# aghasemzadeh/OpenMPL

Hardware: AMD Instinct MI355X
Metric: poses/sec (V=4, J=17, batch=1024 per GPU) fp32 (higher is better)
Workload: dtype f32; 1 GPU; Human3.6M config: V=4 J=17 batch=1024 fp32, CHOSEN flag set, depth 12, DIM 32, heads 8; global_batch=1024, parallelism=single GPU

## Files before the change

openmpl_amd/csrc/spt_native.hip:

```cpp
#include <type_traits>

#include "spt_stage.hpp"

namespace mpl {

constexpr int QS = 100;
constexpr int SPT_LDS_BYTES = (ROWS * XS + ROWS * QS) * 4;

__device__ __forceinline__ int spt_abl(const SptParams& p) {
#ifdef MPL_LAB
    return p.abl;
#else
    return 0;
#endif
}

__device__ __forceinline__ void ln_frags(const float* X, int m, int li, int kq, const float4& g0, const float4& g1,
                                         const float4& b0, const float4& b1, float4& a0, float4& a1) {
    const float* xr = X + (m * 16 + li) * XS + 4 * kq;
    float4 x0 = ld4(xr), x1 = ld4(xr + 16);
    float s = ((x0.x + x0.y) + (x0.z + x0.w)) + ((x1.x + x1.y) + (x1.z + x1.w));
    s = xor16_add(s);
    s = xor32_add(s);
    const float mean = s * (1.0f / 32.0f);
// ... 157 lines not shown
    __device__ __forceinline__ void begin(const mpl_block_weights&, const mpl_block_weights&, bool) {}
};

template <int P, class Weights, class AFrags, class Epilogue>
__device__ __forceinline__ void linear_phase(const Weights& W, int mt, int wave, bool skip, AFrags a_frags, Epilogue epilogue) {
    constexpr int NT = Phase<P>::NT, KH = Phase<P>::KH;
    const int lo = (mt * NT * wave) / NWAVE, hi = (mt * NT * (wave + 1)) / NWAVE;
    for (int m = lo / NT; m * NT < hi && !skip; ++m) {
        float4 a[KH];
        a_frags(m, a);
#pragma unroll
        for (int n = 0; n < NT; ++n) {
            const int u = m * NT + n;
            if (u < lo || u >= hi) continue;
            float4 w[KH];
            float bias;
            W.template tile<P>(n, w, bias);
            f32x4 c = tile_k32(a[0], a[1], w[0], w[1]);
            if constexpr (KH == 4) c = c + tile_k32(a[2], a[3], w[2], w[3]);
            epilogue(m, n, c, bias);
        }
    }
}

template <bool STAGED>
__global__ __launch_bounds__(NTHR, 1) void spt_kernel(const SptParams p) {
    extern __shared__ __attribute__((aligned(1024))) float smem[];
    constexpr int RX = STAGED ? SPT_SMALL_ROWS : ROWS;
    float* WB = smem;
    float* X = smem + (STAGED ? 2 * SPT_WB_FLOATS : 0);
    float* Q = X + RX * XS;

    const int tid = threadIdx.x, lane = tid & 63, wave = __builtin_amdgcn_readfirstlane(tid >> 6);
    const int li = lane & 15, kq = lane >> 4;
    const int view = blockIdx.x % p.V;
    const int b0 = (blockIdx.x / p.V) * p.spw;
    const mpl_spt_set set = p.sets[(p.flags & MPL_F_MULTI_SPT) ? view : 0];
    const float *pose = p.poses[view], *ray = p.rays[view], *cen = p.centers[view];
    const int nl = p.B - b0 < p.spw ? p.B - b0 : p.spw;
    const int rows_live = nl * SJ;
    const int mt = (rows_live + 15) >> 4;

    std::conditional_t<STAGED, StagedWeights, FragWeights> W;
    W.li = li, W.kq = kq;
    if constexpr (STAGED) W.lane = lane;
    mpl_block_weights bw, bw_next;
    if (p.n_apps > 0) {
        bw = set.blocks[p.sched[0] & 0x7f];
        if constexpr (STAGED) stage_block(bw, WB, wave, lane, 0, NWAVE);
        else W.template load<P_QKV>(bw);
        if (STAGED && p.n_apps > 1) bw_next = set.blocks[p.sched[1] & 0x7f];
    }

    spt_embed<false>(p, set, X, tid, b0, pose, ray, cen, nl, mt * 16);
    unsigned char* sched_l = reinterpret_cast<unsigned char*>(WB + SPT_WB_FLOATS + SPT_WB_VEC + 352);
    float* conf_l = WB + SPT_WB_VEC + 352;
    if (STAGED) {
        if (tid < MPL_MAX_APPS) sched_l[tid] = p.sched[tid];
        for (int r = tid; r < rows_live; r += NTHR) {
            const int sq = r / SJ;
            conf_l[r] = pose[((size_t)(b0 + sq) * SJ + (r - sq * SJ)) * 3 + 2];
        }
        asm volatile("s_waitcnt vmcnt(0)" ::: "memory");
    }
    __syncthreads();

    const int abl = spt_abl(p);
    const bool no_mfma = (abl & 4) != 0;
    unsigned long long ph[6] = {0, 0, 0, 0, 0, 0}, tlast = (abl & 16) ? __builtin_amdgcn_s_memtime() : 0;
    auto stamp = [&](int k) {
        if (abl & 16) { const unsigned long long now = __builtin_amdgcn_s_memtime(); ph[k] += now - tlast; tlast = now; }
    };
    float4 g[2], e[2];
    auto a_ln = [&](int m, float4 (&a)[2]) { ln_frags(X, m, li, kq, g[0], g[1], e[0], e[1], a[0], a[1]); };
    auto a_q = [&](int m, auto& a) {
        const float* ar = Q + (m * 16 + li) * QS + 4 * kq;
#pragma unroll
        for (int q = 0; q < (int)(sizeof(a) / sizeof(a[0])); ++q) a[q] = ld4(ar + 16 * q);
    };
    auto add_to_x = [&](int m, int n, const f32x4& c, float b) {
        float* xd = X + (m * 16 + 4 * kq) * XS + n * 16 + li;
#pragma unroll
        for (int r = 0; r < 4; ++r) xd[r * XS] += c[r] + b;
    };
    for (int app = 0; app < p.n_apps; ++app) {
        const bool weighted = ((STAGED ? sched_l[app] : p.sched[app]) & 0x80) != 0;
        const bool more = app + 1 < p.n_apps;
        if (!STAGED && more) bw_next = set.blocks[p.sched[app + 1] & 0x7f];
        if constexpr (STAGED) W.wb = WB + (app & 1) * SPT_WB_FLOATS;
        mpl_block_weights bw_after;

        W.template begin<P_QKV>(bw, bw_next, more);
        W.template ln<P_QKV>(g, e);
        linear_phase<P_QKV>(W, mt, wave, no_mfma, a_ln, [&](int m, int n, const f32x4& c, float b) {
            float* qd = Q + (m * 16 + 4 * kq) * QS + n * 16 + li;
#pragma unroll
            for (int r = 0; r < 4; ++r) qd[r * QS] = c[r] + b;
        });
        __syncthreads();
        stamp(0);

        if (STAGED && more) {
            const int busy = (rows_live * SH + 63) >> 6;
            const int w0 = busy < NWAVE - 1 ? busy : 0;
            stage_block(bw_next, WB + ((app + 1) & 1) * SPT_WB_FLOATS, wave, lane, w0, NWAVE - w0);
            if (app + 2 < p.n_apps) bw_after = set.blocks[sched_l[app + 2] & 0x7f];
        }
        stamp(5);
        for (int pr = tid; pr < rows_live * SH && !(abl & 1); pr += NTHR) {
            const int r = pr >> 3, h = pr & 7;
            const int sq = r / SJ;
            const float* kb = Q + (sq * SJ) * QS + SD + 4 * h;
            const float4 q = ld4(Q + r * QS + 4 * h);
            float sc[SJ];
            float mx = -INFINITY;
#pragma unroll
            for (int j = 0; j < SJ; ++j) {
                const float4 k = ld4(kb + j * QS);
                sc[j] = 0.5f * (fmaf(q.x, k.x, q.y * k.y) + fmaf(q.z, k.z, q.w * k.w));
                mx = fmaxf(mx, sc[j]);
            }
            float l = 0.f;
#pragma unroll
            for (int j = 0; j < SJ; ++j) {
                sc[j] = __expf(sc[j] - mx);
                l += sc[j];
            }
            float inv = 1.0f / l;
            if (weighted) {
                const int b = b0 + sq;
                if (STAGED) inv *= conf_l[r];
                else inv *= (b < p.B) ? pose[((size_t)b * SJ + (r - sq * SJ)) * 3 + 2] : 0.f;
            }
            float4 o = {0.f, 0.f, 0.f, 0.f};
#pragma unroll
            for (int j = 0; j < SJ; ++j) {
                const float4 v = ld4(kb + j * QS + SD);
                const float pj = sc[j] * inv;
                o.x = fmaf(pj, v.x, o.x);
                o.y = fmaf(pj, v.y, o.y);
                o.z = fmaf(pj, v.z, o.z);
                o.w = fmaf(pj, v.w, o.w);
            }
            st4(Q + r * QS + 4 * h, o);
        }
        __syncthreads();
        stamp(1);

        W.template begin<P_PROJ>(bw, bw_next, more);
        linear_phase<P_PROJ>(W, mt, wave, no_mfma, a_q, add_to_x);
        __syncthreads();
        stamp(2);

        W.template begin<P_FC1>(bw, bw_next, more);
        W.template ln<P_FC1>(g, e);
        linear_phase<P_FC1>(W, mt, wave, no_mfma, a_ln, [&](int m, int n, const f32x4& c, float b) {
            float* qd = Q + (m * 16 + 4 * kq) * QS + n * 16 + li;
#pragma unroll
            for (int r = 0; r < 4; ++r) qd[r * QS] = (abl & 2) ? (c[r] + b) : gelu_erf(c[r] + b);
        });
        __syncthreads();
        stamp(3);

        W.template begin<P_FC2>(bw, bw_next, more);
        linear_phase<P_FC2>(W, mt, wave, no_mfma, a_q, add_to_x);
        if (STAGED) asm volatile("s_waitcnt vmcnt(0)" ::: "memory");
        __syncthreads();
        stamp(4);
        bw = bw_next;
        if (STAGED && app + 2 < p.n_apps) bw_next = bw_after;
    }

    if (abl & 16) {
        if (lane == 0 && blockIdx.x < 32) {
            float* o = p.xs + (size_t)(blockIdx.x * NWAVE + wave) * 8;
            for (int k = 0; k < 6; ++k) o[k] = (float)ph[k];
        }
        return;
    }
    spt_epilogue<false>(p, X, tid, view, b0, pose, ray, cen, nl, rows_live);
}

int launch_spt_native(const SptParams& p, int form, int grid, hipStream_t s) {
    if (form == MPL_SPT_STAGED) {
        if (int rc = kernel_lds_once<spt_kernel<true>>(SPT_SMALL_LDS_BYTES)) return rc;
        hipLaunchKernelGGL(spt_kernel<true>, dim3(grid), dim3(NTHR), SPT_SMALL_LDS_BYTES, s, p);
    } else {
        if (int rc = kernel_lds_once<spt_kernel<false>>(SPT_LDS_BYTES)) return rc;
        hipLaunchKernelGGL(spt_kernel<false>, dim3(grid), dim3(NTHR), SPT_LDS_BYTES, s, p);
    }
    return hip_check_launch();
}

}
```

openmpl_amd/csrc/spt_packed.hip:

```cpp
#include "spt_pack.hpp"
#include "spt_stage.hpp"

namespace mpl {

constexpr int ATS = 36;
constexpr int HS = 68;
constexpr int KV_F = SJ * SH * SEQ * 4;
constexpr int SPT3_RING_BYTES = (ROWS * XS + 2 * KV_F + ROWS * ATS) * 4;
constexpr int SPT3_LDS_BYTES = 160 * 1024;
constexpr int SPT3_HID_OFF = 3072;
constexpr int SPT3_Q_OFF = 20480;
static_assert(SPT3_HID_OFF + ROWS * HS <= 2 * KV_F + ROWS * ATS, "HID does not fit its alias");
static_assert((SPT3_HID_OFF + ROWS * HS - 2 * KV_F) * 4 <= SPT3_Q_OFF, "HID reaches into the staged qkv weights");
static_assert(SPT3_Q_OFF + 12 * 1024 <= ROWS * ATS * 4, "staged qkv weights do not fit behind HID in ATT");
static_assert(SPT3_RING_BYTES + 8 * 1024 + 2 * SPT3_NPAR * 4 <= SPT3_LDS_BYTES, "spare LDS too small");

typedef float f32x2 __attribute__((ext_vector_type(2)));

__device__ inline float spt_window_scale(float v) {
    if (!(v > 0.f) || !(v < 3.0e38f)) return 1.0f;
    int e;
    (void)frexpf(32768.0f / v, &e);
    e = e - 1 < -100 ? -100 : (e - 1 > 100 ? 100 : e - 1);
    return ldexpf(1.0f, e);
}

__global__ __launch_bounds__(256) void spt_pack_kernel(const float* __restrict__ qkv_w, const float* __restrict__ qkv_b,
                                                        const float* __restrict__ ln1_w, const float* __restrict__ ln1_b,
                                                        const float* __restrict__ proj_w, const float* __restrict__ proj_b,
                                                        const float* __restrict__ fc1_w, const float* __restrict__ fc1_b,
                                                        const float* __restrict__ ln2_w, const float* __restrict__ ln2_b,
                                                        const float* __restrict__ fc2_w, const float* __restrict__ fc2_b,
                                                        char* __restrict__ dst, int fold_q) {
    __shared__ float Wf[8192];
    __shared__ float cn[SPT_NCOL], sw[SPT_NCOL], bnd[SPT_NCOL], scal[2];
    const int tid = threadIdx.x;
    for (int i = tid; i < 8192; i += 256) {
        float w;
        if (i < 3072) w = qkv_w[i] * ln1_w[i & 31];
        else if (i < 4096) w = proj_w[i - 3072];
        else if (i < 6144) w = fc1_w[i - 4096] * ln2_w[i & 31];
        else w = fc2_w[i - 6144];
        Wf[i] = w;
    }
    __syncthreads();
    if (tid < SPT_NCOL) {
        const int n = tid;
        const float *wr, *raw, *beta = nullptr;
        int K = 32;
        float bias;
        if (n < 96) { wr = Wf + n * 32; raw = qkv_w + n * 32; beta = ln1_b; bias = qkv_b[n]; }
        else if (n < 128) { wr = Wf + 3072 + (n - 96) * 32; raw = proj_w + (n - 96) * 32; bias = proj_b[n - 96]; }
        else if (n < 192) { wr = Wf + 4096 + (n - 128) * 32; raw = fc1_w + (n - 128) * 32; beta = ln2_b; bias = fc1_b[n - 128]; }
        else { wr = Wf + 6144 + (n - 192) * 64; raw = fc2_w + (n - 192) * 64; bias = fc2_b[n - 192]; K = 64; }
        float amax = 0.f;
        double ss = 0.0, c = (double)bias;
        for (int k = 0; k < K; ++k) {
            amax = fmaxf(amax, fabsf(wr[k]));
            ss += (double)wr[k] * (double)wr[k];
            if (beta) c += (double)raw[k] * (double)beta[k];
        }
        float s = 1.0f;
        if (amax > 0.f && amax < 3.0e38f) {
            int e;
            (void)frexpf(amax, &e);
            e = 14 - e;
            e = e < -100 ? -100 : (e > 100 ? 100 : e);
            s = ldexpf(1.0f, e);
// ... 111 lines not shown
            for (int n = 0; n < NCT; ++n) x[n] = res[n];
            if (i + 1 < NM) read_tile(i + 1);
            f32x4 c[NCT];
#pragma unroll
            for (int n = 0; n < NCT; ++n) c[n] = f32x4{0.f, 0.f, 0.f, 0.f};
#pragma unroll
            for (int n = 0; n < NCT; ++n) {
                if (NCT * m + n < LO || NCT * m + n >= HI) continue;
#pragma unroll
                for (int ks = 0; ks < KS; ++ks) c[n] = mfma3(w[n][ks], ah[ks], al[ks], c[n]);
            }
#pragma unroll
            for (int n = 0; n < NCT; ++n) {
                if (NCT * m + n < LO || NCT * m + n >= HI) continue;
                float* dd = d0 + m * 16 * DST + 16 * n;
                if (GELU)
                    st4(dd, float4{gelu_as_scaled(fmaf(c[n][0], sc[n].x, bc[n].x), hs), gelu_as_scaled(fmaf(c[n][1], sc[n].y, bc[n].y), hs),
                                   gelu_as_scaled(fmaf(c[n][2], sc[n].z, bc[n].z), hs), gelu_as_scaled(fmaf(c[n][3], sc[n].w, bc[n].w), hs)});
                else
                    st4(dd, float4{x[n].x + fmaf(c[n][0], sc[n].x, bc[n].x), x[n].y + fmaf(c[n][1], sc[n].y, bc[n].y),
                                   x[n].z + fmaf(c[n][2], sc[n].z, bc[n].z), x[n].w + fmaf(c[n][3], sc[n].w, bc[n].w)});
            }
        }
    }
}
#define SPT_ROLE(W, MTS, KS, LN, GELU, NCT, AST, DST, ...) \
    spt_linear_role<KS, LN, GELU, NCT, AST, DST, ((MTS) * (NCT) * (W)) / NWAVE, ((MTS) * (NCT) * ((W) + 1)) / NWAVE>(__VA_ARGS__)
#define SPT_BY_WAVE(wv, ...)                          \
    switch (wv) {                                     \
        case 0: SPT_ROLE(0, __VA_ARGS__); break;      \
        case 1: SPT_ROLE(1, __VA_ARGS__); break;      \
        case 2: SPT_ROLE(2, __VA_ARGS__); break;      \
        case 3: SPT_ROLE(3, __VA_ARGS__); break;      \
        case 4: SPT_ROLE(4, __VA_ARGS__); break;      \
        case 5: SPT_ROLE(5, __VA_ARGS__); break;      \
        case 6: SPT_ROLE(6, __VA_ARGS__); break;      \
        default: SPT_ROLE(7, __VA_ARGS__); break;     \
    }


template <int SS>
__global__ __launch_bounds__(NTHR, 1) void spt3_kernel(const SptParams p) {
    constexpr int RLIVE = SJ * SS;
    constexpr int MTS = (RLIVE + 15) / 16;
    constexpr int NT = (MTS + 3) / 4;
    extern __shared__ __attribute__((aligned(16))) float smem[];
    float* X = smem;
    float* Kb = smem + ROWS * XS;
    float* Vb = Kb + KV_F;
    float* ATT = Vb + KV_F;
    float* HID = Kb + SPT3_HID_OFF;
    char* S_W = reinterpret_cast<char*>(ATT + ROWS * ATS);
    float* S_PAR = reinterpret_cast<float*>(S_W + 8 * 1024);
    char* R_F1 = reinterpret_cast<char*>(Kb);
    char* R_Q = reinterpret_cast<char*>(ATT) + SPT3_Q_OFF;

    const int tid = threadIdx.x, lane = tid & 63;
    const int wave = __builtin_amdgcn_readfirstlane(tid >> 6);
    const int li = lane & 15, kq = lane >> 4;
    auto phase_sync = [&]() {
        asm volatile("s_waitcnt vmcnt(0)" ::: "memory");
        __syncthreads();
    };
    const int hg = wave & 1, part = wave >> 1;
    const int view = blockIdx.x % p.V;
    const int b0 = (blockIdx.x / p.V) * SS;
    const int sl = li % SS;
    const mpl_spt_set set = p.sets[(p.flags & MPL_F_MULTI_SPT) ? view : 0];
    const float* pose = p.poses[view];
    const float* ray = p.rays[view];
    const float* cen = p.centers[view];

    auto stage_w = [&](char* dst, const unsigned short* pack, int byte_off, int n_pieces) {
        const unsigned l0 = (unsigned)(uintptr_t)(__attribute__((address_space(3))) char*)dst;
        for (int i = wave; i < n_pieces; i += NWAVE)
            ::mpl::dma16(reinterpret_cast<const float*>(reinterpret_cast<const char*>(pack) + byte_off + i * 1024) + lane * 4,
                         l0 + (unsigned)(i * 1024));
    };
    auto load_par = [&](const mpl_block_weights& b) -> float4 {
        if (tid >= SPT3_NPAR / 4) return float4{0.f, 0.f, 0.f, 0.f};
        return ld4(G(reinterpret_cast<const float*>(reinterpret_cast<const char*>(b.qkv_w3) + SPT_PACK_VEC)) + 4 * tid);
    };
    auto store_par = [&](int app_of, const float4& v) {
        if (tid < SPT3_NPAR / 4) st4(S_PAR + (app_of & 1) * SPT3_NPAR + 4 * tid, v);
    };
    mpl_block_weights bw;
    if (p.n_apps > 0) {
        bw = set.blocks[p.sched[0] & 0x7f];
        stage_w(R_Q, bw.qkv_w3, SPT_PACK_QKV, 12);
    }
    const float4 par0 = p.n_apps > 0 ? load_par(bw) : float4{0.f, 0.f, 0.f, 0.f};
    spt_embed<true, SS>(p, set, X, tid, b0, pose, ray, cen, SS, MTS * 16);
    store_par(0, par0);
    phase_sync();

    auto load_w = [&](const char* region, int unit, sf16x8 (&w)[2]) { spt_load_unit(region, unit, lane, w); };
    auto ln_frag = [&](int m, sf16x8& ah, sf16x8& al) {
        const float* xr = X + (m * 16 + li) * XS + 8 * kq;
        spt_ln_split(::mpl::ld4(xr), ::mpl::ld4(xr + 4), ah, al);
    };
    for (int app = 0; app < p.n_apps; ++app) {
        const bool weighted = (p.sched[app] & 0x80) != 0;
        bw = set.blocks[p.sched[app] & 0x7f];
        const unsigned short* pack = bw.qkv_w3;
        const float* par = S_PAR + (app & 1) * SPT3_NPAR;
        stage_w(S_W, pack, SPT_PACK_PROJ, 4);
        {
            sf16x8 wq[3][2];
            float4 bq[3], sq[3];
#pragma unroll
            for (int c = 0; c < 3; ++c) {
                load_w(R_Q, 2 * c + hg, wq[c]);
                bq[c] = ::mpl::ld4(par + SPT_C_QKV + 32 * c + 16 * hg + 4 * kq);
                sq[c] = ::mpl::ld4(par + SPT_NCOL + SPT_C_QKV + 32 * c + 16 * hg + 4 * kq);
            }
            float4 q[NT];
#pragma unroll
            for (int t = 0; t < NT; ++t) {
                q[t] = float4{0.f, 0.f, 0.f, 0.f};
                if (part + 4 * t < MTS && !(p.abl & 8)) {
                    const int m = part + 4 * t;
                    const int j = (16 * m + li) / SS;
                    const bool live = 16 * m + li < RLIVE;
                    sf16x8 ah, al;
                    ln_frag(m, ah, al);
                    const f32x4 z = {0.f, 0.f, 0.f, 0.f};
                    const f32x4 cq = mfma3(wq[0], ah, al, z), ck = mfma3(wq[1], ah, al, z), cv = mfma3(wq[2], ah, al, z);
                    q[t] = float4{fmaf(cq[0], sq[0].x, bq[0].x), fmaf(cq[1], sq[0].y, bq[0].y), fmaf(cq[2], sq[0].z, bq[0].z),
                                  fmaf(cq[3], sq[0].w, bq[0].w)};
                    const int h = 4 * hg + kq;
                    const float kx = fmaf(ck[0], sq[1].x, bq[1].x), ky = fmaf(ck[1], sq[1].y, bq[1].y);
                    const float kz = fmaf(ck[2], sq[1].z, bq[1].z), kw = fmaf(ck[3], sq[1].w, bq[1].w);
                    if (live && j < SJ - 1) {
                        float* kp = Kb + ((((j >> 1) * 2) * SH + h) * SS + sl) * 4 + (j & 1);
                        kp[0] = kx;
                        kp[2] = ky;
                        kp[SH * SS * 4] = kz;
                        kp[SH * SS * 4 + 2] = kw;
                    } else if (live) {
                        st4(Kb + (SJ - 1) * SH * SS * 4 + (h * SS + sl) * 4, float4{kx, ky, kz, kw});
                    }
                    if (live)
                        st4(Vb + ((j * SH + h) * SS + sl) * 4, float4{fmaf(cv[0], sq[2].x, bq[2].x), fmaf(cv[1], sq[2].y, bq[2].y),
                                                                       fmaf(cv[2], sq[2].z, bq[2].z), fmaf(cv[3], sq[2].w, bq[2].w)});
                }
            }
            phase_sync();
            auto attention = [&](auto live_tiles) {
                constexpr int NL = decltype(live_tiles)::value;
                const int h = 4 * hg + kq;
                float sc[NL][SJ];
#pragma unroll
                for (int jp = 0; jp < SJ / 2; ++jp) {
                    const float4 k01 = ::mpl::ld4(Kb + (((jp * 2) * SH + h) * SS + sl) * 4);
                    const float4 k23 = ::mpl::ld4(Kb + (((jp * 2 + 1) * SH + h) * SS + sl) * 4);
                    const f32x2 kx = {k01.x, k01.y}, ky = {k01.z, k01.w}, kz = {k23.x, k23.y}, kw = {k23.z, k23.w};
#pragma unroll
// ... 30 lines not shown
#pragma unroll
                    for (int j = 0; j < SJ; ++j) {
                        sc[t][j] = __builtin_amdgcn_exp2f(sc[t][j] - mx);
                        l += sc[t][j];
                    }
                    inv[t] = __builtin_amdgcn_rcpf(l) * s_att;
                    if (weighted) {
                        const int b = b0 + sl, r = 16 * (part + 4 * t) + li;
                        inv[t] *= (b < p.B && r < RLIVE) ? conf0[3 * (64 / SS) * t] : 0.f;
                    }
                }
                float4 o[NL];
#pragma unroll
                for (int t = 0; t < NL; ++t) o[t] = float4{0.f, 0.f, 0.f, 0.f};
#pragma unroll
                for (int j = 0; j < SJ; ++j) {
                    const float4 v = ::mpl::ld4(Vb + ((j * SH + h) * SS + sl) * 4);
#pragma unroll
                    for (int t = 0; t < NL; ++t) {
                        const float pj = sc[t][j];
                        o[t].x = fmaf(pj, v.x, o[t].x);
                        o[t].y = fmaf(pj, v.y, o[t].y);
                        o[t].z = fmaf(pj, v.z, o[t].z);
                        o[t].w = fmaf(pj, v.w, o[t].w);
                    }
                }
#pragma unroll
                for (int t = 0; t < NL; ++t) {
                    o[t] = float4{o[t].x * inv[t], o[t].y * inv[t], o[t].z * inv[t], o[t].w * inv[t]};
                    if (weighted) {
                        const float big = fmaxf(fmaxf(fabsf(o[t].x), fabsf(o[t].y)), fmaxf(fabsf(o[t].z), fabsf(o[t].w)));
                        if (!(big <= 65000.f)) {
                            const float qn = __builtin_nanf("");
                            o[t] = float4{qn, qn, qn, qn};
                            if (p.err_host) __hip_atomic_fetch_or(p.err_host, 2u, __ATOMIC_RELAXED, __HIP_MEMORY_SCOPE_SYSTEM);
                        }
                    }
                }
#pragma unroll
                for (int t = 0; t < NL; ++t) st4(ATT + ((part + 4 * t) * 16 + li) * ATS + 4 * h, o[t]);
            };
            if (!(p.abl & 1)) {
                if (part + 4 * (NT - 1) < MTS) attention(SptInt<NT>{});
                else if (NT > 1) attention(SptInt<(NT > 1 ? NT - 1 : 1)>{});
            }
        }
        phase_sync();
        stage_w(R_F1, pack, SPT_PACK_FC1, 8);
        if (!(p.abl & 32)) SPT_BY_WAVE(wave, MTS, 1, false, false, 2, ATS, XS, ATT, X, S_W, par, SPT_C_PROJ, 0.f, lane);
        phase_sync();
        stage_w(S_W, pack, SPT_PACK_FC2, 8);
        if (!(p.abl & 64))
            SPT_BY_WAVE(wave, MTS, 1, true, true, 4, XS, HS, X, HID, R_F1, par, SPT_C_FC1, par[2 * SPT_NCOL + 1], lane);
        phase_sync();
        {
            float4 parn = float4{0.f, 0.f, 0.f, 0.f};
            if (app + 1 < p.n_apps) {
                const mpl_block_weights bn = set.blocks[p.sched[app + 1] & 0x7f];
                stage_w(R_Q, bn.qkv_w3, SPT_PACK_QKV, 12);
                parn = load_par(bn);
            }
            if (!(p.abl & 128)) SPT_BY_WAVE(wave, MTS, 2, false, false, 2, HS, XS, HID, X, S_W, par, SPT_C_FC2, 0.f, lane);
            if (app + 1 < p.n_apps) store_par(app + 1, parn);
        }
        phase_sync();
    }
    spt_epilogue<true, SS>(p, X, tid, view, b0, pose, ray, cen, SS, MTS * 16);
}

template <int SS>
static int launch_spt3(const SptParams& p, int grid, hipStream_t s) {
    if (int rc = kernel_lds_once<spt3_kernel<SS>>(SPT3_LDS_BYTES)) return rc;
    hipLaunchKernelGGL(spt3_kernel<SS>, dim3(grid), dim3(NTHR), SPT3_LDS_BYTES, s, p);
    return hip_check_launch();
}

int launch_spt_packed(const SptParams& p, int ss, int grid, hipStream_t s) {
    switch (ss) {
        case 1: return launch_spt3<1>(p, grid, s);
        case 2: return launch_spt3<2>(p, grid, s);
        case 4: return launch_spt3<4>(p, grid, s);
        case 8: return launch_spt3<8>(p, grid, s);
        case 16: return launch_spt3<16>(p, grid, s);
        default: return MPL_E_INVALID;
    }
}

}
```

openmpl_amd/csrc/spt_stage.hpp:

```cpp
#pragma once
#include "common.hpp"

namespace mpl {

constexpr int SJ = 17;
constexpr int SD = 32;
constexpr int SH = 8;
constexpr int SEQ = 16;
constexpr int ROWS = SEQ * SJ;
constexpr int XS = 36;
constexpr int NTHR = 512;
constexpr int NWAVE = NTHR / 64;
constexpr int SPT_SMALL_SPW = 8;

struct SptParams {
    const float* poses[MPL_MAX_VIEWS];
    const float* rays[MPL_MAX_VIEWS];
    const float* centers[MPL_MAX_VIEWS];
    const mpl_spt_set* sets;
    const float *snorm_w, *snorm_b;
    const float *pos3d_embed, *pos3d_view, *pos3d_lin_w, *pos3d_lin_b;
    const float *ray_w, *ray_b, *cfpt_w, *cfpt_b;
    float* xs;
    int B, V, in_ch, n_apps;
    unsigned flags;
    int c3;
    int spw;
    int abl;
    unsigned* err_host;
    unsigned char sched[MPL_MAX_APPS];
};

int launch_spt_native(const SptParams& p, int form, int grid, hipStream_t s);
int launch_spt_packed(const SptParams& p, int ss, int grid, hipStream_t s);

typedef const __attribute__((address_space(1))) float* gfp;
__device__ __forceinline__ gfp G(const float* p) { return (gfp)p; }
__device__ __forceinline__ float4 ld4(gfp p) {
    typedef float v4 __attribute__((ext_vector_type(4)));
    const v4 t = *reinterpret_cast<const __attribute__((address_space(1))) v4*>(p);
    return make_float4(t.x, t.y, t.z, t.w);
}

template <bool TM, int SS = SEQ>
__device__ __forceinline__ void row_to_sj(int r, int& sq, int& j) {
    if (TM) { j = r / SS; sq = r % SS; }
    else { sq = r / SJ; j = r - sq * SJ; }
}

template <bool TM, int SS = SEQ>
__device__ __forceinline__ void spt_embed(const SptParams& p, const mpl_spt_set& set, float* X, int tid, int b0,
                                          const float* pose, const float* ray, const float* cen, int nseq = SEQ, int nrows = ROWS) {
    for (int idx = tid; idx < nrows * SD; idx += NTHR) {
        const int r = idx >> 5, c = idx & 31;
        int sq, j;
        row_to_sj<TM, SS>(r, sq, j);
        const int b = b0 + sq;
        float x = 0.f;
        if (b < p.B && sq < nseq && j < SJ) {
            const float* in = pose + ((size_t)b * SJ + j) * 3;
            const float* we = set.embed_w + c * p.in_ch;
            x = set.embed_b[c] + we[0] * in[0] + we[1] * in[1];
            if (p.in_ch == 3) x += we[2] * in[2];
            if (p.flags & MPL_F_CONF_ADD) x += set.conf_w[c] * in[2] + set.conf_b[c];
            if (p.flags & MPL_F_CONF_MULT) x *= set.conf_w[c] * in[2] + set.conf_b[c];
            x += set.pos_embed[j * SD + c];
            if (p.flags & MPL_F_POS3D_SPATIAL) {
                if (p.flags & MPL_F_POS3D_LEARN) {
                    x += p.pos3d_embed[j * p.c3 + c];
                } else {
                    const float* rr = ray + ((size_t)b * SJ + j) * 3;
                    const float* cc = cen + (size_t)b * 3;
                    const float vx = rr[0] - cc[0], vy = rr[1] - cc[1], vz = rr[2] - cc[2];
                    const float nrm = fmaxf(sqrtf(vx * vx + vy * vy + vz * vz), 1e-12f);
                    const float* wl = p.pos3d_lin_w + c * 3;
                    x += p.pos3d_lin_b[c] + wl[0] * (vx / nrm) + wl[1] * (vy / nrm) + wl[2] * (vz / nrm);
                }
            }
        }
        X[r * XS + c] = x;
    }
}

template <bool TM, int SS = SEQ>
__device__ __forceinline__ void spt_epilogue(const SptParams& p, const float* X, int tid, int view, int b0, const float* pose,
                                             const float* ray, const float* cen, int nseq = SEQ, int nrows = ROWS) {
    const bool to_rays = (p.flags & MPL_F_POS3D_TO_RAYS) && (p.flags & MPL_F_RAYS_TOKEN);
    const bool ray_tok = !(p.flags & MPL_F_POS3D_TO_RAYS) && (p.flags & MPL_F_RAYS_TOKEN);
    const int cw = to_rays ? 2 * SD : SD;
    const int Df = SJ * SD * ((p.flags & MPL_F_RAYS_TOKEN) ? 2 : 1);
    for (int r = tid; r < nrows; r += NTHR) {
        int sq, j;
        row_to_sj<TM, SS>(r, sq, j);
        const int b = b0 + sq;
        if (b >= p.B || sq >= nseq || j >= SJ) continue;
        const float* xr = X + r * XS;
        float v[SD];
        float s = 0.f;
#pragma unroll
        for (int c = 0; c < SD; c += 4) {
            const float4 t = ld4(xr + c);
            v[c] = t.x; v[c + 1] = t.y; v[c + 2] = t.z; v[c + 3] = t.w;
            s += (t.x + t.y) + (t.z + t.w);
        }
        const float mean = s * (1.0f / 32.0f);
        float ss = 0.f;
#pragma unroll
        for (int c = 0; c < SD; ++c) {
            v[c] -= mean;
            ss = fmaf(v[c], v[c], ss);
        }
        const float rstd = 1.0f / sqrtf(ss * (1.0f / 32.0f) + 1e-6f);
        const float conf = pose[((size_t)b * SJ + j) * 3 + 2];
        float dx = 0.f, dy = 0.f, dz = 0.f, nx = 0.f, ny = 0.f, nz = 0.f;
        const bool need_dir = (p.flags & MPL_F_RAYS_TOKEN) ||
                              (!(p.flags & MPL_F_POS3D_SPATIAL) && !(p.flags & MPL_F_POS3D_LEARN));
        if (need_dir) {
            const float* rr = ray + ((size_t)b * SJ + j) * 3;
            const float* cc = cen + (size_t)b * 3;
            dx = rr[0] - cc[0]; dy = rr[1] - cc[1]; dz = rr[2] - cc[2];
            const float nrm = fmaxf(sqrtf(dx * dx + dy * dy + dz * dz), 1e-12f);
            nx = dx / nrm; ny = dy / nrm; nz = dz / nrm;
        }
        auto pos3d = [=](int c) -> float {
            if (p.flags & MPL_F_POS3D_SPATIAL) return p.pos3d_view[j * p.c3 + c];
            if (p.flags & MPL_F_POS3D_LEARN) return p.pos3d_embed[j * p.c3 + c];
            const float* wl = p.pos3d_lin_w + c * 3;
            return p.pos3d_lin_b[c] + wl[0] * nx + wl[1] * ny + wl[2] * nz;
        };
        auto ray_emb = [=](int c) -> float {
            const float* wr = p.ray_w + c * 3;
            return p.ray_b[c] + wr[0] * dx + wr[1] * dy + wr[2] * dz;
        };
        float* orow = p.xs + ((size_t)b * p.V + view) * Df;
        float* o1 = orow + j * cw;
#pragma unroll
        for (int c = 0; c < SD; c += 4) {
            float t[4];
#pragma unroll
            for (int q = 0; q < 4; ++q) {
                float y = v[c + q] * rstd * p.snorm_w[c + q] + p.snorm_b[c + q];
                if (p.flags & MPL_F_CONF_IN_FPT) y += p.cfpt_w[c + q] * conf + p.cfpt_b[c + q];
                t[q] = y + pos3d(c + q);
            }
            st4(o1 + c, float4{t[0], t[1], t[2], t[3]});
        }
        if (to_rays) {
#pragma unroll
            for (int c = 0; c < SD; c += 4) {
                float t[4];
#pragma unroll
                for (int q = 0; q < 4; ++q) t[q] = ray_emb(c + q) + pos3d(SD + c + q);
                st4(o1 + SD + c, float4{t[0], t[1], t[2], t[3]});
            }
        } else if (ray_tok) {
            float* o2 = orow + (SJ + j) * SD;
#pragma unroll
            for (int c = 0; c < SD; c += 4) st4(o2 + c, float4{ray_emb(c), ray_emb(c + 1), ray_emb(c + 2), ray_emb(c + 3)});
        }
    }
}

}
```

Measured before the change: 879,200 poses/s.

## Restructure SPT embed/epilogue for wider parallelism and precompute schedule pointers in LDS

Rewrites the embed stage so each lane holds per-channel weights in registers and processes several rows with batched, prefetched global loads, specialised at compile time by positional-encoding mode. Splits the epilogue into two passes: per-row LayerNorm statistics go to LDS scratch, then 8 threads per row each write a 4-wide slice, so one row is no longer handled serially by a single thread. In the packed kernel, the per-application weight-pack pointers and schedule bytes are resolved once into LDS and read back as scalars, which removes the repeated global lookups of the block table inside the loop. The cost is extra LDS scratch, an added barrier in the epilogue, and higher register pressure.

```diff
diff --git a/openmpl_amd/csrc/spt_native.hip b/openmpl_amd/csrc/spt_native.hip
--- a/openmpl_amd/csrc/spt_native.hip
+++ b/openmpl_amd/csrc/spt_native.hip
@@ -233,6 +233,9 @@
         if (STAGED && p.n_apps > 1) bw_next = set.blocks[p.sched[1] & 0x7f];
     }
 
+    static_assert(MPL_MAX_APPS <= 64, "one lane per scheduled application");
+    unsigned sched_v = 0;
+    if (!STAGED && lane < p.n_apps) sched_v = p.sched[lane];
     spt_embed<false>(p, set, X, tid, b0, pose, ray, cen, nl, mt * 16);
     unsigned char* sched_l = reinterpret_cast<unsigned char*>(WB + SPT_WB_FLOATS + SPT_WB_VEC + 352);
     float* conf_l = WB + SPT_WB_VEC + 352;
@@ -245,6 +248,7 @@
         asm volatile("s_waitcnt vmcnt(0)" ::: "memory");
     }
     __syncthreads();
+    auto sched_of = [&](int a) -> unsigned { return STAGED ? (unsigned)sched_l[a] : (unsigned)__builtin_amdgcn_readlane((int)sched_v, a); };
 
     const int abl = spt_abl(p);
     const bool no_mfma = (abl & 4) != 0;
@@ -265,9 +269,9 @@
         for (int r = 0; r < 4; ++r) xd[r * XS] += c[r] + b;
     };
     for (int app = 0; app < p.n_apps; ++app) {
-        const bool weighted = ((STAGED ? sched_l[app] : p.sched[app]) & 0x80) != 0;
+        const bool weighted = (sched_of(app) & 0x80) != 0;
         const bool more = app + 1 < p.n_apps;
-        if (!STAGED && more) bw_next = set.blocks[p.sched[app + 1] & 0x7f];
+        if (!STAGED && more) bw_next = set.blocks[sched_of(app + 1) & 0x7f];
         if constexpr (STAGED) W.wb = WB + (app & 1) * SPT_WB_FLOATS;
         mpl_block_weights bw_after;
 
@@ -359,7 +363,7 @@
         }
         return;
     }
-    spt_epilogue<false>(p, X, tid, view, b0, pose, ray, cen, nl, rows_live);
+    spt_epilogue<false>(p, X, Q, tid, view, b0, pose, ray, cen, nl, rows_live);
 }
 
 int launch_spt_native(const SptParams& p, int form, int grid, hipStream_t s) {
diff --git a/openmpl_amd/csrc/spt_packed.hip b/openmpl_amd/csrc/spt_packed.hip
--- a/openmpl_amd/csrc/spt_packed.hip
+++ b/openmpl_amd/csrc/spt_packed.hip
@@ -13,7 +13,8 @@
 static_assert(SPT3_HID_OFF + ROWS * HS <= 2 * KV_F + ROWS * ATS, "HID does not fit its alias");
 static_assert((SPT3_HID_OFF + ROWS * HS - 2 * KV_F) * 4 <= SPT3_Q_OFF, "HID reaches into the staged qkv weights");
 static_assert(SPT3_Q_OFF + 12 * 1024 <= ROWS * ATS * 4, "staged qkv weights do not fit behind HID in ATT");
-static_assert(SPT3_RING_BYTES + 8 * 1024 + 2 * SPT3_NPAR * 4 <= SPT3_LDS_BYTES, "spare LDS too small");
+static_assert(SPT3_RING_BYTES + 8 * 1024 + 2 * SPT3_NPAR * 4 + MPL_MAX_APPS * 16 <= SPT3_LDS_BYTES, "spare LDS too small");
+static_assert((2 * SPT3_NPAR * 4) % 16 == 0, "the schedule entries behind the parameters are read as 16-byte words");
 
 typedef float f32x2 __attribute__((ext_vector_type(2)));
 
@@ -231,6 +232,7 @@
     float* HID = Kb + SPT3_HID_OFF;
     char* S_W = reinterpret_cast<char*>(ATT + ROWS * ATS);
     float* S_PAR = reinterpret_cast<float*>(S_W + 8 * 1024);
+    uint4* S_SCH = reinterpret_cast<uint4*>(S_PAR + 2 * SPT3_NPAR);
     char* R_F1 = reinterpret_cast<char*>(Kb);
     char* R_Q = reinterpret_cast<char*>(ATT) + SPT3_Q_OFF;
 
@@ -242,7 +244,11 @@
         __syncthreads();
     };
     const int hg = wave & 1, part = wave >> 1;
-    const int view = blockIdx.x % p.V;
+    int view_v = blockIdx.x % p.V;
+    asm("" : "+v"(view_v));
+    const int view = __builtin_amdgcn_readfirstlane(view_v);
+    unsigned sched_e = 0;
+    if (tid < p.n_apps) sched_e = p.sched[tid];
     const int b0 = (blockIdx.x / p.V) * SS;
     const int sl = li % SS;
     const mpl_spt_set set = p.sets[(p.flags & MPL_F_MULTI_SPT) ? view : 0];
@@ -252,25 +258,42 @@
 
     auto stage_w = [&](char* dst, const unsigned short* pack, int byte_off, int n_pieces) {
         const unsigned l0 = (unsigned)(uintptr_t)(__attribute__((address_space(3))) char*)dst;
+        int ln = lane;
+        asm volatile("" : "+v"(ln));
         for (int i = wave; i < n_pieces; i += NWAVE)
-            ::mpl::dma16(reinterpret_cast<const float*>(reinterpret_cast<const char*>(pack) + byte_off + i * 1024) + lane * 4,
+            ::mpl::dma16(reinterpret_cast<const float*>(reinterpret_cast<const char*>(pack) + byte_off + i * 1024) + ln * 4,
                          l0 + (unsigned)(i * 1024));
     };
-    auto load_par = [&](const mpl_block_weights& b) -> float4 {
+    auto load_par = [&](const unsigned short* pack) -> float4 {
         if (tid >= SPT3_NPAR / 4) return float4{0.f, 0.f, 0.f, 0.f};
-        return ld4(G(reinterpret_cast<const float*>(reinterpret_cast<const char*>(b.qkv_w3) + SPT_PACK_VEC)) + 4 * tid);
+        int t = tid;
+        asm volatile("" : "+v"(t));
+        return ld4(G(reinterpret_cast<const float*>(reinterpret_cast<const char*>(pack) + SPT_PACK_VEC)) + 4 * t);
     };
     auto store_par = [&](int app_of, const float4& v) {
         if (tid < SPT3_NPAR / 4) st4(S_PAR + (app_of & 1) * SPT3_NPAR + 4 * tid, v);
     };
-    mpl_block_weights bw;
+    typedef const __attribute__((address_space(1))) mpl_block_weights* gblock;
+    auto as_pack = [](unsigned lo, unsigned hi) { return reinterpret_cast<const unsigned short*>((uintptr_t)(((unsigned long long)hi << 32) | lo)); };
+    unsigned sched_b = 0;
+    const unsigned short* pack = nullptr;
     if (p.n_apps > 0) {
-        bw = set.blocks[p.sched[0] & 0x7f];
-        stage_w(R_Q, bw.qkv_w3, SPT_PACK_QKV, 12);
-    }
-    const float4 par0 = p.n_apps > 0 ? load_par(bw) : float4{0.f, 0.f, 0.f, 0.f};
+        sched_b = p.sched[0];
+        const unsigned long long a = (unsigned long long)(uintptr_t)((gblock)set.blocks)[sched_b & 0x7f].qkv_w3;
+        pack = as_pack(__builtin_amdgcn_readfirstlane((unsigned)a), __builtin_amdgcn_readfirstlane((unsigned)(a >> 32)));
+        stage_w(R_Q, pack, SPT_PACK_QKV, 12);
+    }
+    const float4 par0 = p.n_apps > 0 ? load_par(pack) : float4{0.f, 0.f, 0.f, 0.f};
+    uint4 entry = {0u, 0u, 0u, 0u};
+    if (tid < p.n_apps) {
+        entry.z = sched_e;
+        const unsigned long long a = (unsigned long long)(uintptr_t)((gblock)set.blocks)[entry.z & 0x7f].qkv_w3;
+        entry.x = (unsigned)a;
+        entry.y = (unsigned)(a >> 32);
+    }
     spt_embed<true, SS>(p, set, X, tid, b0, pose, ray, cen, SS, MTS * 16);
     store_par(0, par0);
+    if (tid < p.n_apps) S_SCH[tid] = entry;
     phase_sync();
 
     auto load_w = [&](const char* region, int unit, sf16x8 (&w)[2]) { spt_load_unit(region, unit, lane, w); };
@@ -279,9 +302,7 @@
         spt_ln_split(::mpl::ld4(xr), ::mpl::ld4(xr + 4), ah, al);
     };
     for (int app = 0; app < p.n_apps; ++app) {
-        const bool weighted = (p.sched[app] & 0x80) != 0;
-        bw = set.blocks[p.sched[app] & 0x7f];
-        const unsigned short* pack = bw.qkv_w3;
+        const bool weighted = (sched_b & 0x80) != 0;
         const float* par = S_PAR + (app & 1) * SPT3_NPAR;
         stage_w(S_W, pack, SPT_PACK_PROJ, 4);
         {
@@ -418,20 +439,28 @@
         stage_w(S_W, pack, SPT_PACK_FC2, 8);
         if (!(p.abl & 64))
             SPT_BY_WAVE(wave, MTS, 1, true, true, 4, XS, HS, X, HID, R_F1, par, SPT_C_FC1, par[2 * SPT_NCOL + 1], lane);
+        const unsigned short* pack_next = nullptr;
+        if (app + 1 < p.n_apps) {
+            const uint4 e = S_SCH[app + 1];
+            pack_next = as_pack(__builtin_amdgcn_readfirstlane(e.x), __builtin_amdgcn_readfirstlane(e.y));
+            sched_b = __builtin_amdgcn_readfirstlane(e.z);
+        }
         phase_sync();
         {
             float4 parn = float4{0.f, 0.f, 0.f, 0.f};
             if (app + 1 < p.n_apps) {
-                const mpl_block_weights bn = set.blocks[p.sched[app + 1] & 0x7f];
-                stage_w(R_Q, bn.qkv_w3, SPT_PACK_QKV, 12);
-                parn = load_par(bn);
+                stage_w(R_Q, pack_next, SPT_PACK_QKV, 12);
+                parn = load_par(pack_next);
             }
             if (!(p.abl & 128)) SPT_BY_WAVE(wave, MTS, 2, false, false, 2, HS, XS, HID, X, S_W, par, SPT_C_FC2, 0.f, lane);
             if (app + 1 < p.n_apps) store_par(app + 1, parn);
         }
+        pack = pack_next;
         phase_sync();
     }
-    spt_epilogue<true, SS>(p, X, tid, view, b0, pose, ray, cen, SS, MTS * 16);
+    int te = tid;
+    asm volatile("" : "+v"(te));
+    spt_epilogue<true, SS>(p, X, Kb, te, view, b0, pose, ray, cen, SS, MTS * 16);
 }
 
 template <int SS>
diff --git a/openmpl_amd/csrc/spt_stage.hpp b/openmpl_amd/csrc/spt_stage.hpp
--- a/openmpl_amd/csrc/spt_stage.hpp
+++ b/openmpl_amd/csrc/spt_stage.hpp
@@ -48,52 +48,177 @@
     else { sq = r / SJ; j = r - sq * SJ; }
 }
 
+
+__device__ __forceinline__ float4 ld4u(gfp p) {
+    typedef float v4u __attribute__((ext_vector_type(4), aligned(4)));
+    const v4u t = *reinterpret_cast<const __attribute__((address_space(1))) v4u*>(p);
+    return make_float4(t.x, t.y, t.z, t.w);
+}
+
+struct SptDir { float dx, dy, dz, nx, ny, nz; };
+__device__ __forceinline__ SptDir spt_dir(const float (&r)[3], const float (&c)[3]) {
+#pragma clang fp contract(off)
+    SptDir d;
+    d.dx = r[0] - c[0]; d.dy = r[1] - c[1]; d.dz = r[2] - c[2];
+    const float nrm = fmaxf(sqrtf(fmaf(d.dx, d.dx, d.dy * d.dy) + d.dz * d.dz), 1e-12f);
+    d.nx = d.dx / nrm; d.ny = d.dy / nrm; d.nz = d.dz / nrm;
+    return d;
+}
+__device__ __forceinline__ float spt_lin3(float b, float w0, float w1, float w2, const SptDir& d) {
+#pragma clang fp contract(off)
+    return (fmaf(w0, d.nx, b) + w1 * d.ny) + w2 * d.nz;
+}
+__device__ __forceinline__ float spt_ray3(float b, float w0, float w1, float w2, const SptDir& d) {
+    return fmaf(w2, d.dz, fmaf(w1, d.dy, fmaf(w0, d.dx, b)));
+}
+
+struct SptEmbedPar { float w0, w1, w2, b, cw, cb, l0, l1, l2, lb; };
+
+template <bool TM, int SS, int N, int M3D>
+__device__ __forceinline__ void spt_embed_rows(const SptParams& p, const mpl_spt_set& set, const SptEmbedPar& e, float* X, int tid, int b0,
+                                               gfp pose, gfp ray, gfp cen, int nseq, int k0, int ntrips) {
+#pragma clang fp contract(off)
+    const int c = tid & 31, r0 = tid >> 5;
+    const bool third = p.in_ch == 3, cadd = (p.flags & MPL_F_CONF_ADD) != 0, cmul = (p.flags & MPL_F_CONF_MULT) != 0;
+    const gfp pos_embed = G(set.pos_embed), pos3d = G(p.pos3d_embed);
+    float in[N][3], pe[N], t3[N], rr[N][3], cc[N][3];
+    bool ok[N];
+#pragma unroll
+    for (int i = 0; i < N; ++i) {
+        int sq, j;
+        row_to_sj<TM, SS>(r0 + 16 * (k0 + i), sq, j);
+        const int b = b0 + sq;
+        ok[i] = b < p.B && sq < nseq && j < SJ;
+        const int bb = b < p.B ? b : p.B - 1, jj = j < SJ ? j : SJ - 1;
+        const gfp ip = pose + ((size_t)bb * SJ + jj) * 3;
+        in[i][0] = ip[0]; in[i][1] = ip[1]; in[i][2] = ip[2];
+        pe[i] = pos_embed[jj * SD + c];
+        if (M3D == 1) t3[i] = pos3d[jj * p.c3 + c];
+        if (M3D == 2) {
+            const gfp rp = ray + ((size_t)bb * SJ + jj) * 3, cp = cen + (size_t)bb * 3;
+            rr[i][0] = rp[0]; rr[i][1] = rp[1]; rr[i][2] = rp[2];
+            cc[i][0] = cp[0]; cc[i][1] = cp[1]; cc[i][2] = cp[2];
+        }
+    }
+#pragma unroll
+    for (int i = 0; i < N; ++i) {
+        float x = (e.b + e.w0 * in[i][0]) + e.w1 * in[i][1];
+        if (third) x = fmaf(e.w2, in[i][2], x);
+        if (cadd) x = x + fmaf(e.cw, in[i][2], e.cb);
+        if (cmul) x = x * fmaf(e.cw, in[i][2], e.cb);
+        x = x + pe[i];
+        if (M3D == 1) x = x + t3[i];
+        if (M3D == 2) x = x + spt_lin3(e.lb, e.l0, e.l1, e.l2, spt_dir(rr[i], cc[i]));
+        if (k0 + i < ntrips) X[(r0 + 16 * (k0 + i)) * XS + c] = ok[i] ? x : 0.f;
+    }
+}
+template <bool TM, int SS, int M3D, int CH, int K0, int NT>
+__device__ __forceinline__ void spt_embed_static(const SptParams& p, const mpl_spt_set& set, const SptEmbedPar& e, float* X, int tid, int b0,
+                                                 gfp pose, gfp ray, gfp cen, int nseq) {
+    constexpr int N = NT - K0 < CH ? NT - K0 : CH;
+    if constexpr (N > 0) {
+        spt_embed_rows<TM, SS, N, M3D>(p, set, e, X, tid, b0, pose, ray, cen, nseq, K0, NT);
+        spt_embed_static<TM, SS, M3D, CH, K0 + N, NT>(p, set, e, X, tid, b0, pose, ray, cen, nseq);
+    }
+}
+template <bool TM, int SS, int M3D>
+__device__ __forceinline__ void spt_embed_mode(const SptParams& p, const mpl_spt_set& set, const SptEmbedPar& e, float* X, int tid, int b0,
+                                               gfp pose, gfp ray, gfp cen, int nseq, int nrows) {
+    if constexpr (TM) spt_embed_static<TM, SS, M3D, (M3D == 2 ? 8 : 17), 0, (SJ * SS + 15) / 16>(p, set, e, X, tid, b0, pose, ray, cen, nseq);
+    else
+        for (int k0 = 0; 16 * k0 < nrows; k0 += 8) spt_embed_rows<TM, SS, 8, M3D>(p, set, e, X, tid, b0, pose, ray, cen, nseq, k0, nrows >> 4);
+}
+
 template <bool TM, int SS = SEQ>
 __device__ __forceinline__ void spt_embed(const SptParams& p, const mpl_spt_set& set, float* X, int tid, int b0,
                                           const float* pose, const float* ray, const float* cen, int nseq = SEQ, int nrows = ROWS) {
-    for (int idx = tid; idx < nrows * SD; idx += NTHR) {
-        const int r = idx >> 5, c = idx & 31;
+    const int c = tid & 31;
+    const bool spatial = (p.flags & MPL_F_POS3D_SPATIAL) != 0, learn = (p.flags & MPL_F_POS3D_LEARN) != 0;
+    SptEmbedPar e = {0.f, 0.f, 0.f, 0.f, 0.f, 0.f, 0.f, 0.f, 0.f, 0.f};
+    const gfp we = G(set.embed_w) + c * p.in_ch;
+    e.w0 = we[0]; e.w1 = we[1];
+    if (p.in_ch == 3) e.w2 = we[2];
+    e.b = G(set.embed_b)[c];
+    if (p.flags & (MPL_F_CONF_ADD | MPL_F_CONF_MULT)) { e.cw = G(set.conf_w)[c]; e.cb = G(set.conf_b)[c]; }
+    if (spatial && !learn) {
+        const gfp wl = G(p.pos3d_lin_w) + c * 3;
+        e.l0 = wl[0]; e.l1 = wl[1]; e.l2 = wl[2];
+        e.lb = G(p.pos3d_lin_b)[c];
+    }
+    if (!spatial) spt_embed_mode<TM, SS, 0>(p, set, e, X, tid, b0, G(pose), G(ray), G(cen), nseq, nrows);
+    else if (learn) spt_embed_mode<TM, SS, 1>(p, set, e, X, tid, b0, G(pose), G(ray), G(cen), nseq, nrows);
+    else spt_embed_mode<TM, SS, 2>(p, set, e, X, tid, b0, G(pose), G(ray), G(cen), nseq, nrows);
+}
+
+template <bool TM, int SS = SEQ>
+__device__ __forceinline__ void spt_epilogue(const SptParams& p, const float* X, float* stat, int tid, int view, int b0, const float* pose_,
+                                             const float* ray_, const float* cen_, int nseq = SEQ, int nrows = ROWS) {
+#pragma clang fp contract(off)
+    constexpr int NK = TM ? (((SJ * SS + 15) / 16) * 16 + 63) / 64 : (ROWS + 63) / 64;
+    const gfp pose = G(pose_), ray = G(ray_), cen = G(cen_);
+    const bool spatial = (p.flags & MPL_F_POS3D_SPATIAL) != 0, learn = (p.flags & MPL_F_POS3D_LEARN) != 0;
+    const bool rtok = (p.flags & MPL_F_RAYS_TOKEN) != 0, cfpt = (p.flags & MPL_F_CONF_IN_FPT) != 0;
+    const bool to_rays = (p.flags & MPL_F_POS3D_TO_RAYS) && rtok;
+    const bool ray_tok = !(p.flags & MPL_F_POS3D_TO_RAYS) && rtok;
+    const bool lin = !spatial && !learn;
+    const bool need_dir = rtok || lin;
+    const int cw = to_rays ? 2 * SD : SD;
+    const int Df = SJ * SD * (rtok ? 2 : 1);
+    const int q4 = 4 * (tid & 7), r0 = tid >> 3;
+
+    const float4 zero4 = {0.f, 0.f, 0.f, 0.f};
+    const float4 sw = ld4u(G(p.snorm_w) + q4), sb = ld4u(G(p.snorm_b) + q4);
+    float4 fw = zero4, fb = zero4, rb = zero4, lb[2] = {zero4, zero4};
+    float4 lw[2][3] = {{zero4, zero4, zero4}, {zero4, zero4, zero4}}, rw[3] = {zero4, zero4, zero4};
+    if (cfpt) { fw = ld4u(G(p.cfpt_w) + q4); fb = ld4u(G(p.cfpt_b) + q4); }
+    if (lin) {
+#pragma unroll
+        for (int h = 0; h < 2; ++h) {
+            if (h == 1 && !to_rays) break;
+            const gfp w = G(p.pos3d_lin_w) + (h * SD + q4) * 3;
+            lw[h][0] = ld4u(w); lw[h][1] = ld4u(w + 4); lw[h][2] = ld4u(w + 8);
+            lb[h] = ld4u(G(p.pos3d_lin_b) + h * SD + q4);
+        }
+    }
+    if (rtok) {
+        const gfp w = G(p.ray_w) + q4 * 3;
+        rw[0] = ld4u(w); rw[1] = ld4u(w + 4); rw[2] = ld4u(w + 8);
+        rb = ld4u(G(p.ray_b) + q4);
+    }
+    const gfp tbl = G(spatial ? p.pos3d_view : p.pos3d_embed);
+    bool ok[NK];
+    int jr[NK], br[NK];
+    float conf[NK], rr[NK][3], cc[NK][3];
+    float4 tb[NK][2];
+#pragma unroll
+    for (int k = 0; k < NK; ++k) {
+        const int r = r0 + 64 * k;
         int sq, j;
         row_to_sj<TM, SS>(r, sq, j);
         const int b = b0 + sq;
-        float x = 0.f;
-        if (b < p.B && sq < nseq && j < SJ) {
-            const float* in = pose + ((size_t)b * SJ + j) * 3;
-            const float* we = set.embed_w + c * p.in_ch;
-            x = set.embed_b[c] + we[0] * in[0] + we[1] * in[1];
-            if (p.in_ch == 3) x += we[2] * in[2];
-            if (p.flags & MPL_F_CONF_ADD) x += set.conf_w[c] * in[2] + set.conf_b[c];
-            if (p.flags & MPL_F_CONF_MULT) x *= set.conf_w[c] * in[2] + set.conf_b[c];
-            x += set.pos_embed[j * SD + c];
-            if (p.flags & MPL_F_POS3D_SPATIAL) {
-                if (p.flags & MPL_F_POS3D_LEARN) {
-                    x += p.pos3d_embed[j * p.c3 + c];
-                } else {
-                    const float* rr = ray + ((size_t)b * SJ + j) * 3;
-                    const float* cc = cen + (size_t)b * 3;
-                    const float vx = rr[0] - cc[0], vy = rr[1] - cc[1], vz = rr[2] - cc[2];
-                    const float nrm = fmaxf(sqrtf(vx * vx + vy * vy + vz * vz), 1e-12f);
-                    const float* wl = p.pos3d_lin_w + c * 3;
-                    x += p.pos3d_lin_b[c] + wl[0] * (vx / nrm) + wl[1] * (vy / nrm) + wl[2] * (vz / nrm);
-                }
-            }
-        }
-        X[r * XS + c] = x;
-    }
-}
-
-template <bool TM, int SS = SEQ>
-__device__ __forceinline__ void spt_epilogue(const SptParams& p, const float* X, int tid, int view, int b0, const float* pose,
-                                             const float* ray, const float* cen, int nseq = SEQ, int nrows = ROWS) {
-    const bool to_rays = (p.flags & MPL_F_POS3D_TO_RAYS) && (p.flags & MPL_F_RAYS_TOKEN);
-    const bool ray_tok = !(p.flags & MPL_F_POS3D_TO_RAYS) && (p.flags & MPL_F_RAYS_TOKEN);
-    const int cw = to_rays ? 2 * SD : SD;
-    const int Df = SJ * SD * ((p.flags & MPL_F_RAYS_TOKEN) ? 2 : 1);
+        ok[k] = r < nrows && b < p.B && sq < nseq && j < SJ;
+        const int bb = b < p.B ? b : p.B - 1, jj = j < SJ ? j : SJ - 1;
+        jr[k] = jj; br[k] = bb;
+        conf[k] = 0.f;
+        if (cfpt) conf[k] = pose[((size_t)bb * SJ + jj) * 3 + 2];
+        if (need_dir) {
+            const gfp rp = ray + ((size_t)bb * SJ + jj) * 3, cp = cen + (size_t)bb * 3;
+            rr[k][0] = rp[0]; rr[k][1] = rp[1]; rr[k][2] = rp[2];
+            cc[k][0] = cp[0]; cc[k][1] = cp[1]; cc[k][2] = cp[2];
+        } else {
+            rr[k][0] = rr[k][1] = rr[k][2] = cc[k][0] = cc[k][1] = cc[k][2] = 0.f;
+        }
+        tb[k][0] = tb[k][1] = zero4;
+        if (!lin) {
+            tb[k][0] = ld4u(tbl + jj * p.c3 + q4);
+            if (to_rays) tb[k][1] = ld4u(tbl + jj * p.c3 + SD + q4);
+        }
+    }
+
     for (int r = tid; r < nrows; r += NTHR) {
         int sq, j;
         row_to_sj<TM, SS>(r, sq, j);
-        const int b = b0 + sq;
-        if (b >= p.B || sq >= nseq || j >= SJ) continue;
+        if (b0 + sq >= p.B || sq >= nseq || j >= SJ) continue;
         const float* xr = X + r * XS;
         float v[SD];
         float s = 0.f;
@@ -103,62 +228,56 @@
             v[c] = t.x; v[c + 1] = t.y; v[c + 2] = t.z; v[c + 3] = t.w;
             s += (t.x + t.y) + (t.z + t.w);
         }
-        const float mean = s * (1.0f / 32.0f);
         float ss = 0.f;
 #pragma unroll
         for (int c = 0; c < SD; ++c) {
-            v[c] -= mean;
+            v[c] = fmaf(s, -1.0f / 32.0f, v[c]);
             ss = fmaf(v[c], v[c], ss);
         }
-        const float rstd = 1.0f / sqrtf(ss * (1.0f / 32.0f) + 1e-6f);
-        const float conf = pose[((size_t)b * SJ + j) * 3 + 2];
-        float dx = 0.f, dy = 0.f, dz = 0.f, nx = 0.f, ny = 0.f, nz = 0.f;
-        const bool need_dir = (p.flags & MPL_F_RAYS_TOKEN) ||
-                              (!(p.flags & MPL_F_POS3D_SPATIAL) && !(p.flags & MPL_F_POS3D_LEARN));
-        if (need_dir) {
-            const float* rr = ray + ((size_t)b * SJ + j) * 3;
-            const float* cc = cen + (size_t)b * 3;
-            dx = rr[0] - cc[0]; dy = rr[1] - cc[1]; dz = rr[2] - cc[2];
-            const float nrm = fmaxf(sqrtf(dx * dx + dy * dy + dz * dz), 1e-12f);
-            nx = dx / nrm; ny = dy / nrm; nz = dz / nrm;
-        }
-        auto pos3d = [=](int c) -> float {
-            if (p.flags & MPL_F_POS3D_SPATIAL) return p.pos3d_view[j * p.c3 + c];
-            if (p.flags & MPL_F_POS3D_LEARN) return p.pos3d_embed[j * p.c3 + c];
-            const float* wl = p.pos3d_lin_w + c * 3;
-            return p.pos3d_lin_b[c] + wl[0] * nx + wl[1] * ny + wl[2] * nz;
+        stat[2 * r] = s;
+        stat[2 * r + 1] = 1.0f / sqrtf(fmaf(ss, 1.0f / 32.0f, 1e-6f));
+    }
+    __syncthreads();
+
+#pragma unroll
+    for (int k = 0; k < NK; ++k) {
+        if (!ok[k]) continue;
+        const int r = r0 + 64 * k;
+        const float4 xq = ld4(X + r * XS + q4);
+        const float s = stat[2 * r], rstd = stat[2 * r + 1];
+        SptDir d = {0.f, 0.f, 0.f, 0.f, 0.f, 0.f};
+        if (need_dir) d = spt_dir(rr[k], cc[k]);
+        const float x[4] = {xq.x, xq.y, xq.z, xq.w};
+        const float w[4] = {sw.x, sw.y, sw.z, sw.w}, bs[4] = {sb.x, sb.y, sb.z, sb.w};
+        const float fwa[4] = {fw.x, fw.y, fw.z, fw.w}, fba[4] = {fb.x, fb.y, fb.z, fb.w};
+        const float rba[4] = {rb.x, rb.y, rb.z, rb.w};
+        const float rwa[12] = {rw[0].x, rw[0].y, rw[0].z, rw[0].w, rw[1].x, rw[1].y, rw[1].z, rw[1].w, rw[2].x, rw[2].y, rw[2].z, rw[2].w};
+        auto pos3d = [&](int h, int i) -> float {
+            if (!lin) { const float4 t = tb[k][h]; return i == 0 ? t.x : i == 1 ? t.y : i == 2 ? t.z : t.w; }
+            const float la[12] = {lw[h][0].x, lw[h][0].y, lw[h][0].z, lw[h][0].w, lw[h][1].x, lw[h][1].y, lw[h][1].z, lw[h][1].w,
+                                  lw[h][2].x, lw[h][2].y, lw[h][2].z, lw[h][2].w};
+            const float ba[4] = {lb[h].x, lb[h].y, lb[h].z, lb[h].w};
+            return spt_lin3(ba[i], la[3 * i], la[3 * i + 1], la[3 * i + 2], d);
         };
-        auto ray_emb = [=](int c) -> float {
-            const float* wr = p.ray_w + c * 3;
-            return p.ray_b[c] + wr[0] * dx + wr[1] * dy + wr[2] * dz;
-        };
-        float* orow = p.xs + ((size_t)b * p.V + view) * Df;
-        float* o1 = orow + j * cw;
-#pragma unroll
-        for (int c = 0; c < SD; c += 4) {
-            float t[4];
-#pragma unroll
-            for (int q = 0; q < 4; ++q) {
-                float y = v[c + q] * rstd * p.snorm_w[c + q] + p.snorm_b[c + q];
-                if (p.flags & MPL_F_CONF_IN_FPT) y += p.cfpt_w[c + q] * conf + p.cfpt_b[c + q];
-                t[q] = y + pos3d(c + q);
-            }
-            st4(o1 + c, float4{t[0], t[1], t[2], t[3]});
-        }
+        auto ray_emb = [&](int i) -> float { return spt_ray3(rba[i], rwa[3 * i], rwa[3 * i + 1], rwa[3 * i + 2], d); };
+        float* orow = p.xs + ((size_t)br[k] * p.V + view) * Df;
+        float* o1 = orow + jr[k] * cw + q4;
+        float t[4];
+#pragma unroll
+        for (int i = 0; i < 4; ++i) {
+            float y = fmaf(fmaf(s, -1.0f / 32.0f, x[i]) * rstd, w[i], bs[i]);
+            if (cfpt) y = y + fmaf(fwa[i], conf[k], fba[i]);
+            t[i] = y + pos3d(0, i);
+        }
+        st4(o1, float4{t[0], t[1], t[2], t[3]});
         if (to_rays) {
 #pragma unroll
-            for (int c = 0; c < SD; c += 4) {
-                float t[4];
-#pragma unroll
-                for (int q = 0; q < 4; ++q) t[q] = ray_emb(c + q) + pos3d(SD + c + q);
-                st4(o1 + SD + c, float4{t[0], t[1], t[2], t[3]});
-            }
+            for (int i = 0; i < 4; ++i) t[i] = ray_emb(i) + pos3d(1, i);
+            st4(o1 + SD, float4{t[0], t[1], t[2], t[3]});
         } else if (ray_tok) {
-            float* o2 = orow + (SJ + j) * SD;
-#pragma unroll
-            for (int c = 0; c < SD; c += 4) st4(o2 + c, float4{ray_emb(c), ray_emb(c + 1), ray_emb(c + 2), ray_emb(c + 3)});
-        }
-    }
-}
-
-}
+            st4(orow + (SJ + jr[k]) * SD + q4, float4{ray_emb(0), ray_emb(1), ray_emb(2), ray_emb(3)});
+        }
+    }
+}
+
+}
```

Result: no change. 885,700 poses/s, median of 6 (+0.7%).
